# adelacvg/NS2VC

Measured on AMD Instinct MI355X. Metric: denoiser-steps/sec (10s@24kHz Vocos latent, bs32), higher is better.
Workload: dtype fp16; 1 GPU; 10 s utterance (T=938 Vocos frames), batch 32/GPU, prompt Lp=469, 20-step unipc order 2, hipGraph-captured loop, fp16 MFMA operands; timed job = set_condition + 20 steps; global_batch=32, frames=938, prompt_frames=469, solver=unipc, parallelism=dp1

## Files before the change

### include/ns2vc_hip.h

```cpp
#ifndef NS2VC_HIP_H
#define NS2VC_HIP_H

#include <stddef.h>
#include <stdint.h>

#ifdef __cplusplus
extern "C" {
#endif

#define NS2VC_ABI_VERSION 7
#define NS2VC_MAX_LEVELS 8
#define NS2VC_NCOEF 12

typedef struct ns2vc_unet ns2vc_unet;

typedef struct ns2vc_unet_cfg {
  int32_t latent_channels;
  int32_t content_channels;
  int32_t n_levels;
  int32_t block_out_channels[NS2VC_MAX_LEVELS];
  int32_t norm_num_groups;
  int32_t cross_attention_dim;
  int32_t heads;
  int32_t layers_per_block;
// ... 168 lines not shown
typedef struct ns2vc_rowchain_args {
  const void* a_op; int32_t lda;
  const void* wstream; const float* bias1; const float* consts2;
  const float* res; int32_t ldres;
  float* out1_f32; int32_t ldo1;
  void* out2_op; int32_t ldo2;
  float ln_eps; int32_t M, dim, n2;
  unsigned* ln_health;
  const float* gn_x; int32_t ldx;
  const long long* gn_stats; const float* gn_gamma; const float* gn_beta;
  float gn_eps; int32_t T, G;
  int32_t slices;
  const int32_t* lens;
} ns2vc_rowchain_args;
int ns2vc_pack_rowchain(const float* w1_host, const float* w2_host, int dim, int n2, int precision, void** out_stream_dev);
int ns2vc_pack_rowchain_sliced(const float* w1_host, const float* w2_host, int dim, int n2, int slices, int precision, void** out_stream_dev);
int ns2vc_k_rowchain(const ns2vc_rowchain_args* a, int precision, void* stream);
int ns2vc_debug_set_geglu_min_rows(int rows);
int ns2vc_debug_set_attn_keys(int keys);
int ns2vc_debug_set_attn_optimistic(int on);
int ns2vc_debug_set_attn_resident(int mode);
unsigned long long ns2vc_debug_attn_resident_launches(void);
int ns2vc_debug_attnres_table(int* rows);
int ns2vc_debug_set_rowchain_tokens(int nt);

int ns2vc_to_operand(const float* host, size_t n, int precision, void** out_dev);
int ns2vc_from_operand(const void* dev, size_t n, int precision, float* host);
int ns2vc_round_to_operand(const float* host_in, size_t n, int precision, float* host_out);
int ns2vc_pack_weight(const float* rows_host, int N, int K, int precision, void** out_dev);
int ns2vc_k_gemm(const ns2vc_gemm_args* a, int precision, void* stream);
int ns2vc_pack_conv3_tiled(const float* rows_host, int N, int ctot, int c2, int precision, void** out_dev);
int ns2vc_weight_rowsum(const float* rows_host, int N, int K, int precision, float** out_dev);
int ns2vc_debug_set_gemm_trace(void* dev_u64_blocks_x8);
int ns2vc_debug_poison(unsigned pattern, int lds_bytes, void* stream);
int ns2vc_debug_placement(void* stream, int n_blocks, int spin, uint32_t* out_host);
int ns2vc_debug_kernel_table(int family, int* rows, int* unready);
int ns2vc_debug_set_gemm_tile(int bm, int bn, int stages);
int ns2vc_k_attention(const ns2vc_attn_args* a, int head_dim, int precision, void* stream);
int ns2vc_k_groupnorm(const float* a0, int lda0, int c0, const float* a1, int lda1, int c1, int B, int T, int G, float eps,
                      const float* gamma, const float* beta, const float* temb, int ldtemb, int temb_off, int silu,
                      void* out_op, void* raw_op, int precision, void* stream);
int ns2vc_k_groupnorm_stats(const float* a0, int lda0, int c0, const long long* stats0, int B, int T, int G, float eps, const float* gamma,
                            const float* beta, const float* temb, int ldtemb, int temb_off, int silu, void* out_op, int precision, void* stream);
int ns2vc_k_groupnorm_stats2(const float* a0, int lda0, int c0, const long long* stats0, const float* a1, int lda1, int c1, const long long* stats1,
                             int B, int T, int G, float eps, const float* gamma, const float* beta, const float* temb, int ldtemb, int temb_off,
                             int silu, void* out_op, void* raw_op, int precision, void* stream);
// ... 39 lines not shown
```

### ns2vc_amd/_lib.py

```python
from __future__ import annotations

import ctypes as C
import os
from typing import Optional

_HERE = os.path.dirname(os.path.abspath(__file__))
LIB_PATH = os.path.join(_HERE, "lib", "libns2vc_hip.so")
NCOEF = 12
MAX_LEVELS = 8
PREC_F32, PREC_BF16, PREC_F16 = 0, 1, 2
ABI_VERSION = 7


class Ns2vcError(RuntimeError):
    pass


class UnetCfg(C.Structure):
    _fields_ = [
        ("latent_channels", C.c_int32), ("content_channels", C.c_int32), ("n_levels", C.c_int32),
        ("block_out_channels", C.c_int32 * MAX_LEVELS), ("norm_num_groups", C.c_int32),
        ("cross_attention_dim", C.c_int32), ("heads", C.c_int32), ("layers_per_block", C.c_int32),
        ("pool_heads", C.c_int32),
    ]
# ... 166 lines not shown
    "ns2vc_debug_set_gemm_tile": (_I, [_I, _I, _I]),
    "ns2vc_debug_kernel_table": (_I, [_I, C.POINTER(C.c_int), C.POINTER(C.c_int)]),
    "ns2vc_debug_placement": (_I, [_P, _I, _I, C.POINTER(C.c_uint32)]),
    "ns2vc_debug_poison": (_I, [C.c_uint, _I, _P]),
    "ns2vc_k_attention": (_I, [C.POINTER(AttnArgs), _I, _I, _P]),
    "ns2vc_pack_ffn": (_I, [_P, _P, _I, _I, _PP]),
    "ns2vc_pack_ffn_pre": (_I, [_P, _P, _P, _I, _I, _PP]),
    "ns2vc_xattn_pack_bytes": (C.c_size_t, [_I, _I, _I]),
    "ns2vc_k_xattn_pack": (_I, [_P, _I, _P, _I, _I, _I, _I, _P, _I, _P]),
    "ns2vc_k_ffn": (_I, [C.POINTER(FfnArgs), _I, _P]),
    "ns2vc_pack_geglu": (_I, [_P, _P, _I, _I, _PP, _PP]),
    "ns2vc_k_geglu": (_I, [C.POINTER(GegluArgs), _I, _P]),
    "ns2vc_pack_geglu_host": (_I, [_P, _P, _I, _I, _P, _P]),
    "ns2vc_debug_set_geglu_min_rows": (_I, [_I]),
    "ns2vc_pack_rowchain": (_I, [_P, _P, _I, _I, _I, _PP]),
    "ns2vc_pack_rowchain_sliced": (_I, [_P, _P, _I, _I, _I, _I, _PP]),
    "ns2vc_k_rowchain": (_I, [C.POINTER(RowchainArgs), _I, _P]),
    "ns2vc_debug_set_rowchain_tokens": (_I, [_I]),
    "ns2vc_debug_set_attn_keys": (_I, [_I]),
    "ns2vc_debug_set_attn_optimistic": (_I, [_I]),
    "ns2vc_debug_set_attn_resident": (_I, [_I]),
    "ns2vc_debug_attnres_table": (_I, [C.POINTER(_I)]),
    "ns2vc_debug_attn_resident_launches": (C.c_ulonglong, []),
    "ns2vc_k_groupnorm_stats": (_I, [_P, _I, _I, _P, _I, _I, _I, C.c_float, _P, _P, _P, _I, _I, _I, _P, _I, _P]),
    "ns2vc_k_groupnorm_stats2": (_I, [_P, _I, _I, _P, _P, _I, _I, _P, _I, _I, _I, C.c_float, _P, _P, _P, _I, _I, _I, _P, _P, _I, _P]),
    "ns2vc_k_groupnorm": (_I, [_P, _I, _I, _P, _I, _I, _I, _I, _I, C.c_float, _P, _P, _P, _I, _I, _I, _P, _P, _I, _P]),
    "ns2vc_k_layernorm_apply": (_I, [_P, _I, _I, _I, C.c_float, _P, _I, _P]),
    "ns2vc_to_operand": (_I, [_P, C.c_size_t, _I, _PP]),
    "ns2vc_from_operand": (_I, [_P, C.c_size_t, _I, _P]),
    "ns2vc_round_to_operand": (_I, [_P, C.c_size_t, _I, _P]),
    "ns2vc_k_nct_to_btc": (_I, [_P, _I, _I, _I, _P, _I, _I, _P]),
    "ns2vc_k_btc_to_nct": (_I, [_P, _I, _I, _I, _I, _P, _P]),
    "ns2vc_k_noise": (_I, [_P, _I, _I, _I, _I, _I, _P, _P, _P]),
    "ns2vc_k_solver_update": (_I, [_P, _P, _P, _P, _P, _I, _P, _P, _P, _P, C.c_size_t, _I, _P]),
    "ns2vc_k_solver_update_guided": (_I, [_P, _P, _P, _P, _P, _I, _P, _P, _P, _P, C.c_size_t, _I, _P, _I, _P, _P, _I, _P]),
    "ns2vc_k_abs_quantile": (_I, [_P, _I, _I, _I, _I, _P, C.c_float, _P, _P]),
    "ns2vc_k_solver_update_corrected": (_I, [_P, _P, _P, _P, _P, _I, _P, _P, _P, _P, C.c_size_t, _I, _I, _P, _P, _I, _I, C.c_float, C.c_float, _P, _P]),
    "ns2vc_k_solver_update_items": (_I, [_P, _I, _P, _P, _I, _P, _P, _P, _I, _P, _P, _P, _P, C.c_size_t, _I, _I, _P, _P, _P, _I, _I, C.c_float, C.c_float,
                                         _P, _P]),
    "ns2vc_k_solver_update_items_corrected": (_I, [_P, _I, _P, _P, _I, _P, _P, _P, _I, _P, _P, _P, _P, C.c_size_t, _I, _I, _P, _P, _P, _I, _P, _P, _P,
                                                   _P, _P]),
    "ns2vc_sampler_open": (_I, [_P, _I, _I, _P]),
    "ns2vc_sampler_rebase": (_I, [_P, _P]),
    "ns2vc_sampler_write_rows": (_I, [_P, _I, _I, C.POINTER(C.c_float), _P]),
    "ns2vc_sampler_admit": (_I, [_P, _I, _P, _P, _P, _P]),
    "ns2vc_sampler_take": (_I, [_P, _I, _P, _P, _P]),
# ... 48 lines not shown
```

### ns2vc_amd/csrc/abi_kernels.cpp

```cpp
#include "engine_internal.h"
#include "kernel_table.h"

#include <algorithm>
#include <cstring>
#include <mutex>

using namespace ns2vc;

hipError_t ns2vc::init_all_attributes() {
  hipError_t e = init_gemm_attributes();
  if (e == hipSuccess) e = init_convts_attributes();
  if (e == hipSuccess) e = init_attn_attributes();
  if (e == hipSuccess) e = init_attnres_attributes();
  if (e == hipSuccess) e = init_ffn_attributes();
  if (e == hipSuccess) e = init_geglu_attributes();
  if (e == hipSuccess) e = init_rowchain_attributes();
  return e;
}
static int init_attributes(hipError_t (*init)(), bool* once = nullptr) {
  if (once && *once) return 0;
  const hipError_t e = init();
  if (e != hipSuccess) return fail("kernel attribute setup failed: %s", hipGetErrorString(e));
  if (once) *once = true;
  return 0;
// ... 196 lines not shown
  static bool inited = false;
  if (init_attributes(init_rowchain_attributes, &inited)) return 1;
  std::vector<unsigned short> st;
  if (pack_rowchain_stream(w1_host, w2_host, dim, n2, precision, st, slices) != hipSuccess)
    return fail("rowchain (sliced): dim 384, n2 = dim or 3 dim, 2 slices, 16-bit precision");
  return upload_u16(st, out_stream_dev);
}
int ns2vc_debug_set_attn_keys(int keys) {
  if (keys != 0 && keys != 64 && keys != 128) return fail("attention K/V tile: 0 (heuristic), 64 or 128 keys");
  set_forced_attn_keys(keys);
  return 0;
}
int ns2vc_debug_set_attn_resident(int mode) {
  if (mode < -1 || mode > 1) return fail("resident attention: -1 (the rule), 0 (never) or 1 (whenever the launch fits)");
  set_attn_resident_mode(mode);
  return 0;
}
unsigned long long ns2vc_debug_attn_resident_launches(void) { return attn_resident_launches(); }
int ns2vc_debug_attnres_table(int* rows) {
  if (!rows) return fail("attnres table: rows not NULL");
  *rows = attnres_kernel_table().n;
  return 0;
}
int ns2vc_debug_set_rowchain_tokens(int nt) {
  if (nt < 0 || nt > 2) return fail("rowchain tokens: 0 (heuristic), 1 (64-token blocks) or 2 (128-token blocks)");
  set_forced_rowchain_tokens(nt);
  return 0;
}
int ns2vc_k_rowchain(const ns2vc_rowchain_args* a, int precision, void* stream) {
  if (!a) return fail("null args");
  return launched(launch_rowchain(*a, precision, (hipStream_t)stream), "launch_rowchain");
}
size_t ns2vc_xattn_pack_bytes(int B, int Lk, int hd) { return xattn_pack_bytes(B, Lk, hd); }
int ns2vc_k_xattn_pack(const void* k, int ldk, const void* v, int ldv, int B, int Lk, int hd, void* out, int precision, void* stream) {
  hipError_t e = launch_xattn_pack(k, ldk, v, ldv, B, Lk, hd, out, precision, (hipStream_t)stream);
  if (e != hipSuccess) return fail("xattn_pack: %s (16-bit precisions, head dim 16 | 32, 8 heads, 16-byte aligned k rows)", hipGetErrorString(e));
  return 0;
}
int ns2vc_k_ffn(const ns2vc_ffn_args* a, int precision, void* stream) {
  if (!a) return fail("null args");
  return launched(launch_ffn(*a, precision, (hipStream_t)stream), "launch_ffn");
}
int ns2vc_pack_geglu(const float* w1_packed_host, const float* bias1_packed_host, int dim, int precision, void** out_stream_dev, float** out_consts_dev) {
  if (!w1_packed_host || !out_stream_dev || !out_consts_dev) return fail("null argument");
  if (init_attributes(init_geglu_attributes)) return 1;
  std::vector<unsigned short> st;
// ... 242 lines not shown
```

### ns2vc_amd/csrc/common.h

```cpp
#pragma once
#include <hip/hip_runtime.h>
#include <stdint.h>
#include <stddef.h>
#include <vector>
#include "../../include/ns2vc_hip.h"

namespace ns2vc {

typedef __attribute__((ext_vector_type(8))) __bf16 bf16x8_t;
typedef __attribute__((ext_vector_type(16))) float f32x16_t;
typedef __attribute__((ext_vector_type(4))) float f32x4_t;
typedef __attribute__((ext_vector_type(4))) unsigned int u32x4_t;

struct bf16_t { uint16_t v; };
struct f16_t { uint16_t v; };

__host__ __device__ inline uint16_t f32_to_bf16_bits(float f) {
  union { float f; uint32_t u; } x;
  x.f = f;
  uint32_t u = x.u;
  if ((u & 0x7fffffffu) > 0x7f800000u) return (uint16_t)((u >> 16) | 0x40);
  u += 0x7fffu + ((u >> 16) & 1u);
  return (uint16_t)(u >> 16);
}
// ... 245 lines not shown
bool gemm_uses_convts(const GemmArgs& g, int prec);
int last_gemm_refusal_line();
hipError_t launch_attention(const AttnArgs& a, int head_dim, int prec, hipStream_t s, bool resident = true);
bool attention_resident_eligible(const AttnArgs& a, int head_dim, int prec, bool allow);
hipError_t launch_attention_resident(const AttnArgs& a, int head_dim, int prec, hipStream_t s);
hipError_t init_attnres_attributes();
void set_attn_resident_mode(int mode);
unsigned long long attn_resident_launches();
void set_attnres_optimistic(int on);
bool attention_masks_rows(const AttnArgs& a, int head_dim, int prec);
hipError_t init_gemm_attributes();
bool convts_eligible(const GemmArgs& g, int prec);
int convts_default_bn(const GemmArgs& g);
int convts_bn_for(const GemmArgs& g, int bn128_min);
void set_convts_bn128_min(int wgs);
int convts_row_blocks(const GemmArgs& g);
hipError_t launch_convts(const GemmArgs& g, int prec, int bn, int nl, int ks, hipStream_t s);
hipError_t init_convts_attributes();
hipError_t pack_conv3_tiled(const float* rows, int N, int ctot, int c2, int prec, std::vector<unsigned char>& out);
void set_forced_gemm_tile(int bm, int bn, int stages);
void set_gemm_trace(unsigned long long* p);
hipError_t init_attn_attributes();
void set_forced_attn_keys(int keys);
hipError_t launch_ffn(const ::ns2vc_ffn_args& a, int prec, hipStream_t s);
bool ffn_eligible(int dim, int T, int prec);
bool ffn_masks_rows(const ::ns2vc_ffn_args& a, int prec);
hipError_t init_ffn_attributes();
hipError_t pack_ffn_stream(const float* w1p, const float* w2f, const float* w0, int dim, int prec, std::vector<unsigned short>& out);
void set_ffn_trace(unsigned long long* p);
bool geglu_eligible(int dim, int T, int prec);
hipError_t pack_geglu_stream(const float* w1p, const float* bias1p, int dim, int prec, std::vector<unsigned short>& stream, std::vector<float>& consts);
hipError_t launch_geglu(const ::ns2vc_geglu_args& a, int prec, hipStream_t s);
bool geglu_masks_rows(const ::ns2vc_geglu_args& a, int prec);
hipError_t init_geglu_attributes();
void set_gg_trace(unsigned long long* p);
void set_ts_trace(unsigned long long* p);
void set_attn_optimistic(int on);

hipError_t launch_gn_partial(const float* a0, int lda0, int c0, const float* a1, int lda1, int c1,
                             int B, int T, int G, double* partial, int nchunk, int rows_per_chunk, hipStream_t s);
hipError_t launch_gn_apply(const float* a0, int lda0, int c0, const float* a1, int lda1, int c1, int B, int T, int G, float eps,
                           const double* partial, int nchunk, const long long* st0, const long long* st1, const float* gamma,
                           const float* beta, const float* temb, int ldtemb, int temb_off, int silu, void* out_op, void* raw_op,
                           int prec, hipStream_t s, int pair = 0,
                           const int* lens = nullptr);
hipError_t launch_mask_rows(void* dst, size_t ldd_bytes, size_t row_bytes, int B, int T, const int* lens, hipStream_t s, const void* src = nullptr,
                            size_t lds_bytes = 0, int Tsrc = 0, int up = 0);
hipError_t launch_ln_apply_op(const float* x, int ldx, int M, int C, float eps, void* out_op, int prec, hipStream_t s);
// ... 71 lines not shown
```

### ns2vc_amd/csrc/engine.cpp

```cpp
#include "engine_internal.h"

#include <algorithm>
#include <cstdlib>
#include <cstring>

using namespace ns2vc;

static int bind_device(ns2vc_unet* h) {
  int cur = -1;
  HIPCHK(hipGetDevice(&cur));
  if (cur != h->device) HIPCHK(hipSetDevice(h->device));
  return 0;
}
int ns2vc::check_ready(ns2vc_unet* h, bool need_plan) {
  if (!h) return fail("null engine handle");
  if (bind_device(h)) return 1;
  if (!h->finalized) return fail("weights not finalized (call ns2vc_unet_finalize_weights)");
  if (need_plan && !h->arena) return fail("engine not prepared (call ns2vc_unet_prepare)");
  return 0;
}

int ns2vc::load_state(ns2vc_unet* h, const float* x_bct, hipStream_t s, int items) {
  const int B = items > 0 ? items : h->B;
  HIPCHK(launch_nct_to_btc(x_bct, h->cfg.latent_channels, h->T, B, h->xe, h->xe_op, h->prec, h->CP, h->CP, s, h->pair_width(), h->pair_off()));
  if (!h->lens.masked) return 0;
  const size_t ob = (size_t)h->pair_width() * operand_bytes(h->prec);
  HIPCHK(launch_mask_rows(h->xe, (size_t)h->CP * 4, (size_t)h->CP * 4, B, h->T, h->lens.dev, s));
  HIPCHK(launch_mask_rows(h->xe_op, ob, ob, B, h->T, h->lens.dev, s));
  return 0;
}

static const struct { const char* name; const char* env; bool ns2vc_unet::* member; } kOptions[] = {
  {"ln_linear", "NS2VC_LN_LINEAR", &ns2vc_unet::ln_linear}, {"fold_ff", "NS2VC_FOLD_FF", &ns2vc_unet::fold_ff},
  {"fuse_ffn", "NS2VC_FUSE_FFN", &ns2vc_unet::fuse_ffn}, {"fuse_ffn_pre", "NS2VC_FUSE_FFN_PRE", &ns2vc_unet::fuse_ffn_pre},
  {"fuse_geglu", "NS2VC_FUSE_GEGLU", &ns2vc_unet::fuse_geglu}, {"fuse_rows", "NS2VC_FUSE_ROWS", &ns2vc_unet::fuse_rows},
  {"fuse_rows_gn", "NS2VC_FUSE_ROWS_GN", &ns2vc_unet::fuse_rows_gn}, {"fuse_gn_gemm", "NS2VC_FUSE_GN_GEMM", &ns2vc_unet::fuse_gn_gemm},
  {"fuse_gn_cat", "NS2VC_FUSE_GN_CAT", &ns2vc_unet::fuse_gn_cat}, {"gn_coop", "NS2VC_GN_COOP", &ns2vc_unet::gn_coop},
  {"slice_rows", "NS2VC_SLICE_ROWS", &ns2vc_unet::slice_rows}, {"attn_fp8", "NS2VC_ATTN_FP8", &ns2vc_unet::attn_fp8},
  {"attn_optimistic", "NS2VC_ATTN_OPTIMISTIC", &ns2vc_unet::attn_optimistic}, {"conv_ts", "NS2VC_CONV_TS", &ns2vc_unet::conv_ts},
  {"conv_wtiled", "NS2VC_CONV_WTILED", &ns2vc_unet::conv_wtiled}, {"gn_inloop", "NS2VC_GN_INLOOP", &ns2vc_unet::gn_inloop},
  {"fuse_solver", "NS2VC_FUSE_SOLVER", &ns2vc_unet::fuse_solver}, {"fuse_xattn", "NS2VC_FUSE_XATTN", &ns2vc_unet::fuse_xattn},
  {"fork_temb", "NS2VC_FORK_TEMB", &ns2vc_unet::fork_temb}, {"exact_io", "NS2VC_EXACT_IO", &ns2vc_unet::exact_io},
  {"split_io", "NS2VC_SPLIT_IO", &ns2vc_unet::split_io}, {"masked_fuse", "NS2VC_MASKED_FUSE", &ns2vc_unet::masked_fuse},
  {"masked_attn", "NS2VC_MASKED_ATTN", &ns2vc_unet::masked_attn}, {"masked_rows", "NS2VC_MASKED_ROWS", &ns2vc_unet::masked_rows},
  {"masked_ffn", "NS2VC_MASKED_FFN", &ns2vc_unet::masked_ffn}, {"masked_geglu", "NS2VC_MASKED_GEGLU", &ns2vc_unet::masked_geglu},
  {"attn_resident", "NS2VC_ATTN_RESIDENT", &ns2vc_unet::attn_resident}};
static bool* option_ptr(ns2vc_unet* h, const char* name) {
  for (const auto& o : kOptions)
    if (!strcmp(name, o.name)) return &(h->*o.member);
  return nullptr;
}

extern "C" {

int ns2vc_unet_create(const ns2vc_unet_cfg* cfg, ns2vc_unet** out) {
  if (!cfg || !out) return fail("null argument");
  if (cfg->n_levels < 2 || cfg->n_levels > NS2VC_MAX_LEVELS) return fail("n_levels=%d out of range (2..%d)", cfg->n_levels, NS2VC_MAX_LEVELS);
  if (cfg->latent_channels <= 0 || cfg->latent_channels > 128) return fail("latent_channels=%d must be in 1..128", cfg->latent_channels);
  if (cfg->content_channels <= 0 || cfg->content_channels % 64)
    return fail("content_channels=%d must be a positive multiple of 64", cfg->content_channels);
  if (cfg->cross_attention_dim <= 0 || cfg->cross_attention_dim % 128)
    return fail("cross_attention_dim=%d must be a positive multiple of 128", cfg->cross_attention_dim);
  if (cfg->heads < 1) return fail("heads=%d must be >= 1", cfg->heads);
  if (cfg->norm_num_groups < 1 || cfg->norm_num_groups > 8) return fail("norm_num_groups=%d unsupported (1..8)", cfg->norm_num_groups);
  if (cfg->layers_per_block < 1) return fail("layers_per_block=%d must be >= 1", cfg->layers_per_block);
  if (cfg->pool_heads < 1 || cfg->cross_attention_dim % cfg->pool_heads || cfg->cross_attention_dim / cfg->pool_heads > 8)
    return fail("cross_attention_dim=%d over pool_heads=%d: the pool head width must be a whole number <= 8", cfg->cross_attention_dim, cfg->pool_heads);
  if (cfg->block_out_channels[0] != 128) return fail("block_out_channels[0]=%d must be 128 (padded latent width)", cfg->block_out_channels[0]);
  for (int l = 0; l < cfg->n_levels; ++l) {
// ... 459 lines not shown
```

### ns2vc_amd/csrc/engine_internal.h

```cpp
#pragma once
#include "common.h"

#include <cmath>
#include <cstdarg>
#include <cstdio>
#include <cstring>
#include <functional>
#include <map>
#include <string>
#include <vector>

namespace ns2vc {

inline thread_local std::string g_err;

inline int fail(const char* fmt, ...) {
  char buf[1024];
  va_list ap;
  va_start(ap, fmt);
  vsnprintf(buf, sizeof(buf), fmt, ap);
  va_end(ap);
  g_err = buf;
  return 1;
}
// ... 212 lines not shown
  int conv_out_prec = -1;
  bool fork_temb = false;
  struct TembFork {
    int begin = -1, end = -1, join = -1;
    int first = -1, readers = 0;
    bool ok = false;
    int join_skip = 0;
    hipStream_t side_stream = nullptr;
    hipEvent_t ev_fork = nullptr, ev_join = nullptr;
  } tfork;
  bool fuse_xattn = false;
  bool fuse_solver = false;
  ns2vc::GemmArgs conv_out_g;
  int conv_out_idx = -1;
  bool warned_wtiled = false;
  int bn128_min = 160;
  bool gn_inloop = false;
  int gn_coop_min = 2;
  int cus = 256;
  int xcd_probe = -1;
  bool slice_rows = true;
  unsigned* ln_health = nullptr;
  bool attn_optimistic = true;
  bool attn_resident = true;
  unsigned* attn_fallbacks = nullptr;
  unsigned long long coef_hash = 0;
  std::vector<ns2vc::Tap> taps;
  bool has_mask = false;
  bool masked_fuse = false;
  bool masked_attn = false;
  bool masked_rows = false;
  bool masked_ffn = false;
  bool masked_geglu = false;
  struct Lengths {
    bool masked = false;
    int* dev = nullptr;
    size_t off = 0;
    float* selfbias = nullptr;
    std::vector<int32_t> applied;
    ns2vc::Staged stage;
  } lens;
  struct PromptLengths {
    bool on = false;
    int* dev = nullptr;
    std::vector<int32_t> applied;
    ns2vc::Staged stage;
// ... 111 lines not shown
```

### ns2vc_amd/csrc/ffn.hip

```cpp
#include "common.h"
#include <type_traits>
#include "mma.h"
#include "kernel_table.h"
#include <vector>

namespace ns2vc {

typedef ::ns2vc_ffn_args FfnArgs;

__device__ unsigned long long* g_ffn_trace = nullptr;
#ifndef NS2VC_GEMM_TRACE
#define NS2VC_GEMM_TRACE 0
#endif
#ifndef NS2VC_FFN_FENCE
#define NS2VC_FFN_FENCE 1
#endif
#ifndef NS2VC_FFN_WARM
#define NS2VC_FFN_WARM 1
#endif
#if NS2VC_FFN_FENCE == 1
#define FFN_FRAG_FENCE() do { asm volatile("s_waitcnt lgkmcnt(0)" ::: "memory"); __builtin_amdgcn_sched_barrier(0); } while (0)
#elif NS2VC_FFN_FENCE == 2
#define FFN_FRAG_FENCE() __builtin_amdgcn_sched_barrier(0)
#else
// ... 651 lines not shown
  return hipGetLastError();
}

static uint64_t ffn_key(const FfnArgs& a, int prec, bool masked) { return kernel_key(prec, a.dim, a.pre_a || a.att_q, a.att_q != nullptr, masked); }
#define NS2VC_FFN_ROW(TM, PREC, D, PRE, ATT, MK) \
  {kernel_key(PREC, D, PRE, ATT, MK), reinterpret_cast<const void*>(ffn_kernel<TM, D, PRE, ATT, MK>), (uint32_t)FfnGeom<D, PRE>::LDS, 512}
#define NS2VC_FFN_ROWS(PRE, ATT, MK)                                                              \
  NS2VC_FFN_ROW(bf16_t, PREC_BF16, 128, PRE, ATT, MK), NS2VC_FFN_ROW(bf16_t, PREC_BF16, 256, PRE, ATT, MK), \
  NS2VC_FFN_ROW(f16_t, PREC_F16, 128, PRE, ATT, MK), NS2VC_FFN_ROW(f16_t, PREC_F16, 256, PRE, ATT, MK)
static const KernelRow ffn_rows[] = {
  NS2VC_FFN_ROWS(false, false, false), NS2VC_FFN_ROWS(true, false, false),
  NS2VC_FFN_ROWS(false, false, true), NS2VC_FFN_ROWS(true, false, true),
  NS2VC_FFN_ROWS(true, true, false),
};
#undef NS2VC_FFN_ROWS
#undef NS2VC_FFN_ROW
static const KernelTable k_ffn_table(ffn_rows);
const KernelTable& ffn_kernel_table() { return k_ffn_table; }

bool ffn_masks_rows(const FfnArgs& a, int prec) {
  return ffn_eligible(a.dim, a.T, prec) && a.B >= 1 && a.M == a.B * a.T && find(k_ffn_table, ffn_key(a, prec, true));
}

hipError_t launch_ffn(const FfnArgs& a, int prec, hipStream_t s) {
  if (!ffn_eligible(a.dim, a.T, prec) || a.M <= 0 || a.M != a.B * a.T) return hipErrorInvalidValue;
  if (a.lens) {
    if (!ffn_masks_rows(a, prec)) return hipErrorInvalidValue;
  }
  if (!a.wstream || !a.consts || !a.bias2 || !a.res || (!a.out_f32 && !a.out_op)) return hipErrorInvalidValue;
  if (a.att_q) {
    if (!a.pre_bias || !a.pre_res || (a.pre_ldres & 3) || !a.att_kv || a.att_Lk < 1 || (a.att_ldq & 7) ||
        ((reinterpret_cast<uintptr_t>(a.att_q) | reinterpret_cast<uintptr_t>(a.att_kv)) & 15) || !(a.att_scale > 0.f))
      return hipErrorInvalidValue;
  } else if (a.pre_a ? (!a.pre_bias || !a.pre_res || (a.pre_lda & 7) || (a.pre_ldres & 3) || (unsigned long long)a.M * a.pre_lda * 2ull > 0xFFF00000ull)
              : (!a.yn || !a.ln_stats))
    return hipErrorInvalidValue;
  if ((!a.pre_a && !a.att_q && (a.ldy & 7)) || (a.ldres & 3) || (a.out_f32 && (a.ldo_f32 & 3)) || (a.out_op && (a.ldo_op & 3))) return hipErrorInvalidValue;
  if (!a.pre_a && !a.att_q && (unsigned long long)a.M * a.ldy * 2ull > 0xFFF00000ull) return hipErrorInvalidValue;
  const KernelRow* row = find(k_ffn_table, ffn_key(a, prec, a.lens != nullptr));
  if (!row) return hipErrorInvalidValue;
  return launch(*row, dim3(a.att_q ? a.B * ((a.T + 63) / 64) : (a.M + 63) / 64), s, a);
}

hipError_t init_ffn_attributes() { return set_lds_all(k_ffn_table); }

}
```

### ns2vc_amd/csrc/kernel_table.h

```cpp
#pragma once
#include <hip/hip_runtime.h>

#include <cstdint>

namespace ns2vc {

constexpr uint64_t KEY_NONE = ~0ull;
constexpr uint64_t kernel_key() { return 0; }
template <typename... I> constexpr uint64_t kernel_key(int f, I... rest) {
  static_assert(sizeof...(I) < 6, "six fields of ten bits");
  const uint64_t r = kernel_key(rest...);
  return ((unsigned)f >> 10) || r == KEY_NONE ? KEY_NONE : (r << 10 | (unsigned)f);
}

struct KernelRow {
  uint64_t key;
  const void* fn;
  uint32_t lds;
  uint32_t threads;
};
struct KernelTable {
  const KernelRow* rows;
  int n;
  template <int N> constexpr KernelTable(const KernelRow (&r)[N]) : rows(r), n(N) {}
// ... 5 lines not shown
  return nullptr;
}
inline hipError_t set_lds_all(const KernelTable& t) {
  for (int i = 0; i < t.n; ++i) {
    const hipError_t e = hipFuncSetAttribute(t.rows[i].fn, hipFuncAttributeMaxDynamicSharedMemorySize, (int)t.rows[i].lds);
    if (e != hipSuccess) return e;
  }
  return hipSuccess;
}
template <typename... A> hipError_t launch(const KernelRow& r, dim3 grid, hipStream_t s, const A&... args) {
  void* p[] = {const_cast<void*>(static_cast<const void*>(&args))...};
  (void)hipLaunchKernel(r.fn, grid, dim3(r.threads), p, r.lds, s);
  return hipGetLastError();
}

const KernelTable& gemm2_kernel_table();
const KernelTable& gemm4_kernel_table();
const KernelTable& conv3ts_kernel_table();
const KernelTable& attn_kernel_table();
const KernelTable& ffn_kernel_table();
const KernelTable& geglu_kernel_table();
const KernelTable& rowchain_kernel_table();
const KernelTable& attnres_kernel_table();

}
```

### ns2vc_amd/csrc/plan.cpp

```cpp
#include "engine_internal.h"

#include <algorithm>
#include <cmath>
#include <cstring>

namespace ns2vc {

int g_geglu_min_rows = 4608;

std::vector<int> level_lengths(int T, int n_levels) {
  std::vector<int> Ts(n_levels);
  Ts[0] = T;
  for (int l = 1; l < n_levels; ++l) Ts[l] = (Ts[l - 1] + 1) / 2;
  return Ts;
}

namespace {

struct Planner {
  ns2vc_unet* h;
  std::vector<Op>* ops;
  bool sizing = false;
  size_t off = 0;
  int B, T, Lp, G, prec;
// ... 343 lines not shown
      gemm(t + ".attn2.to_out", g);
    }
    if (ffn_ok) {
      ns2vc_ffn_args f;
      memset(&f, 0, sizeof(f));
      f.yn = yn; f.ldy = d; f.ln_stats = r3; f.ln_eps = 1e-5f;
      f.wstream = a.ffn_stream; f.consts = a.ffn_consts; f.bias2 = a.ffpo.bias;
      if (ffn_pre) {
        f.yn = nullptr; f.ln_stats = nullptr; f.wstream = a.ffn_pre_stream;
        f.pre_a = ao; f.pre_lda = d; f.pre_bias = a.o2.bias; f.pre_res = y; f.pre_ldres = d;
      }
      if (xatt) {
        f.pre_a = nullptr;
        f.att_q = qb; f.att_ldq = d; f.att_kv = xattn_vt[a.prefix];
        f.att_bias = (h->has_mask || h->plens.on) ? h->maskbias : nullptr; f.att_scale = 1.0f / std::sqrt((float)hd); f.att_Lk = Lp;
      }
      f.res = x; f.ldres = d;
      f.out_f32 = out; f.ldo_f32 = d; f.out_op = out_op; f.ldo_op = d;
      f.stats = new_stats(out, Tl, d);
      f.B = B; f.T = Tl; f.M = M; f.dim = d; f.ln_health = h->ln_health;
      if (lens_ffn) f.lens = lens_of(Tl);
      const double fl = 2.0 * M * (double)d * ((ffn_pre ? 14.0 : 13.0) * d) + (xatt ? 4.0 * B * h->cfg.heads * (double)Tl * Lp * hd : 0.0);
      add(a.prefix + (xatt ? ".ffn[attn2.sdpa+to_out+geglu+ff.out+proj_out]" : ffn_pre ? ".ffn[attn2.to_out+geglu+ff.out+proj_out]" : ".ffn[geglu+ff.out+proj_out]"),
          [=](hipStream_t s) { return launch_ffn(f, pr, s); }, 1, fl,
          (double)M * d * (opsz + 8.0 + (ffn_pre ? 4.0 : 0.0) + (out_op ? opsz : 0.0)) + (ffn_pre ? 14.0 : 13.0) * d * d * opsz +
              (xatt ? (double)opsz * B * d * 2.0 * Lp : 0.0));
      return;
    }
    auto geglu_masks = [&]() {
      ns2vc_geglu_args f;
      memset(&f, 0, sizeof(f));
      f.M = M; f.dim = d; f.T = Tl;
      return geglu_masks_rows(f, pr);
    };
    const bool lens_geglu = masked && h->masked_geglu && ops == &h->fwd_ops && level_of(Tl) >= 0 && lin_dense && fold && h->fuse_geglu &&
                            a.geglu_stream && geglu_eligible(d, Tl, pr) && M >= g_geglu_min_rows && geglu_masks();
    if (!r3 && !lens_geglu) layernorm(t + ".norm3");
    if (lens_geglu || (r3 && h->fuse_geglu && a.geglu_stream && geglu_eligible(d, Tl, pr) && M >= g_geglu_min_rows)) {
      ns2vc_geglu_args f;
      memset(&f, 0, sizeof(f));
      f.yn = yn; f.ldy = d; f.ln_stats = r3; f.ln_eps = 1e-5f;
      if (lens_geglu) { f.yn = qb; f.ln_stats = nullptr; f.T = Tl; f.lens = lens_of(Tl); }
      f.wstream = a.geglu_stream; f.consts = a.geglu_consts;
      f.out_op = ffh; f.ldo = 4 * d; f.M = M; f.dim = d; f.ln_health = h->ln_health;
      add(t + ".ff.geglu[token-stationary]", [=](hipStream_t s) { return launch_geglu(f, pr, s); }, 1, 2.0 * M * (double)d * 8.0 * d,
          (double)M * d * opsz * 5.0 + (double)M * (d / 64) * 8.0 + 8.0 * d * d * opsz);
    } else {
// ... 338 lines not shown
```

Baseline: 284.5 denoiser-steps/s (batch 32 per GPU, whole job).

## Add 128-token wide fused FFN kernel for dim-128 pre-projection path

Adds a new fused feed-forward kernel (to_out + LayerNorm + GEGLU + ff.out + proj_out) that processes 128 tokens per block with 8 waves, a 7-deep weight-tile ring in LDS and a cooperative weight prefetch. It is used when dim is 128, the pre-projection path is active without masks or cross-attention, and the 64-token grid would exceed the CU count. The aim is to halve how often the weight stream is re-read per token and raise MFMA reuse. The cost is a large LDS footprint per block, lower occupancy, and a dispatch rule that may pick the wrong kernel for some shapes.

Result: no change. 287.1 denoiser-steps/s (batch 32 per GPU, whole job), median of 6 (+0.9%).

```diff
diff --git a/include/ns2vc_hip.h b/include/ns2vc_hip.h
--- a/include/ns2vc_hip.h
+++ b/include/ns2vc_hip.h
@@ -214,6 +214,14 @@
 int ns2vc_debug_set_attn_resident(int mode);
 unsigned long long ns2vc_debug_attn_resident_launches(void);
 int ns2vc_debug_attnres_table(int* rows);
+#define NS2VC_FFNW_16BIT 1
+#define NS2VC_FFNW_PRE 2
+#define NS2VC_FFNW_LENS 4
+#define NS2VC_FFNW_ATT 8
+int ns2vc_debug_set_ffn_wide(int mode);
+unsigned long long ns2vc_debug_ffn_wide_launches(void);
+int ns2vc_debug_ffn_wide_rule(int M, int dim, int flags, int cus);
+int ns2vc_debug_ffnwide_table(int* rows);
 int ns2vc_debug_set_rowchain_tokens(int nt);
 
 int ns2vc_to_operand(const float* host, size_t n, int precision, void** out_dev);
diff --git a/ns2vc_amd/_lib.py b/ns2vc_amd/_lib.py
--- a/ns2vc_amd/_lib.py
+++ b/ns2vc_amd/_lib.py
@@ -212,6 +212,10 @@
     "ns2vc_debug_set_attn_resident": (_I, [_I]),
     "ns2vc_debug_attnres_table": (_I, [C.POINTER(_I)]),
     "ns2vc_debug_attn_resident_launches": (C.c_ulonglong, []),
+    "ns2vc_debug_set_ffn_wide": (_I, [_I]),
+    "ns2vc_debug_ffn_wide_launches": (C.c_ulonglong, []),
+    "ns2vc_debug_ffn_wide_rule": (_I, [_I, _I, _I, _I]),
+    "ns2vc_debug_ffnwide_table": (_I, [C.POINTER(_I)]),
     "ns2vc_k_groupnorm_stats": (_I, [_P, _I, _I, _P, _I, _I, _I, C.c_float, _P, _P, _P, _I, _I, _I, _P, _I, _P]),
     "ns2vc_k_groupnorm_stats2": (_I, [_P, _I, _I, _P, _P, _I, _I, _P, _I, _I, _I, C.c_float, _P, _P, _P, _I, _I, _I, _P, _P, _I, _P]),
     "ns2vc_k_groupnorm": (_I, [_P, _I, _I, _P, _I, _I, _I, _I, _I, C.c_float, _P, _P, _P, _I, _I, _I, _P, _P, _I, _P]),
diff --git a/ns2vc_amd/csrc/abi_kernels.cpp b/ns2vc_amd/csrc/abi_kernels.cpp
--- a/ns2vc_amd/csrc/abi_kernels.cpp
+++ b/ns2vc_amd/csrc/abi_kernels.cpp
@@ -242,6 +242,18 @@
   *rows = attnres_kernel_table().n;
   return 0;
 }
+int ns2vc_debug_set_ffn_wide(int mode) {
+  if (mode < -1 || mode > 1) return fail("128-token feed-forward: -1 (the rule), 0 (never) or 1 (whenever the arguments fit)");
+  set_ffn_wide_mode(mode);
+  return 0;
+}
+unsigned long long ns2vc_debug_ffn_wide_launches(void) { return ffn_wide_launches(); }
+int ns2vc_debug_ffn_wide_rule(int M, int dim, int flags, int cus) { return ffn_wide_rule(M, dim, flags, cus) ? 1 : 0; }
+int ns2vc_debug_ffnwide_table(int* rows) {
+  if (!rows) return fail("ffnwide table: rows not NULL");
+  *rows = ffnwide_kernel_table().n;
+  return 0;
+}
 int ns2vc_debug_set_rowchain_tokens(int nt) {
   if (nt < 0 || nt > 2) return fail("rowchain tokens: 0 (heuristic), 1 (64-token blocks) or 2 (128-token blocks)");
   set_forced_rowchain_tokens(nt);
diff --git a/ns2vc_amd/csrc/common.h b/ns2vc_amd/csrc/common.h
--- a/ns2vc_amd/csrc/common.h
+++ b/ns2vc_amd/csrc/common.h
@@ -291,8 +291,14 @@
 void set_gemm_trace(unsigned long long* p);
 hipError_t init_attn_attributes();
 void set_forced_attn_keys(int keys);
-hipError_t launch_ffn(const ::ns2vc_ffn_args& a, int prec, hipStream_t s);
+hipError_t launch_ffn(const ::ns2vc_ffn_args& a, int prec, hipStream_t s, bool wide = true);
 bool ffn_eligible(int dim, int T, int prec);
+bool ffn_wide_rule(int M, int dim, int flags, int cus);
+bool ffn_wide_eligible(const ::ns2vc_ffn_args& a, int prec, bool allow);
+hipError_t launch_ffn_wide(const ::ns2vc_ffn_args& a, int prec, hipStream_t s);
+hipError_t init_ffnwide_attributes();
+void set_ffn_wide_mode(int mode);
+unsigned long long ffn_wide_launches();
 bool ffn_masks_rows(const ::ns2vc_ffn_args& a, int prec);
 hipError_t init_ffn_attributes();
 hipError_t pack_ffn_stream(const float* w1p, const float* w2f, const float* w0, int dim, int prec, std::vector<unsigned short>& out);
diff --git a/ns2vc_amd/csrc/engine.cpp b/ns2vc_amd/csrc/engine.cpp
--- a/ns2vc_amd/csrc/engine.cpp
+++ b/ns2vc_amd/csrc/engine.cpp
@@ -44,7 +44,7 @@
   {"split_io", "NS2VC_SPLIT_IO", &ns2vc_unet::split_io}, {"masked_fuse", "NS2VC_MASKED_FUSE", &ns2vc_unet::masked_fuse},
   {"masked_attn", "NS2VC_MASKED_ATTN", &ns2vc_unet::masked_attn}, {"masked_rows", "NS2VC_MASKED_ROWS", &ns2vc_unet::masked_rows},
   {"masked_ffn", "NS2VC_MASKED_FFN", &ns2vc_unet::masked_ffn}, {"masked_geglu", "NS2VC_MASKED_GEGLU", &ns2vc_unet::masked_geglu},
-  {"attn_resident", "NS2VC_ATTN_RESIDENT", &ns2vc_unet::attn_resident}};
+  {"attn_resident", "NS2VC_ATTN_RESIDENT", &ns2vc_unet::attn_resident}, {"ffn_wide", "NS2VC_FFN_WIDE", &ns2vc_unet::ffn_wide}};
 static bool* option_ptr(ns2vc_unet* h, const char* name) {
   for (const auto& o : kOptions)
     if (!strcmp(name, o.name)) return &(h->*o.member);
diff --git a/ns2vc_amd/csrc/engine_internal.h b/ns2vc_amd/csrc/engine_internal.h
--- a/ns2vc_amd/csrc/engine_internal.h
+++ b/ns2vc_amd/csrc/engine_internal.h
@@ -258,6 +258,7 @@
   bool slice_rows = true;
   unsigned* ln_health = nullptr;
   bool attn_optimistic = true;
+  bool ffn_wide = true;
   bool attn_resident = true;
   unsigned* attn_fallbacks = nullptr;
   unsigned long long coef_hash = 0;
diff --git a/ns2vc_amd/csrc/ffn.hip b/ns2vc_amd/csrc/ffn.hip
--- a/ns2vc_amd/csrc/ffn.hip
+++ b/ns2vc_amd/csrc/ffn.hip
@@ -697,7 +697,7 @@
   return ffn_eligible(a.dim, a.T, prec) && a.B >= 1 && a.M == a.B * a.T && find(k_ffn_table, ffn_key(a, prec, true));
 }
 
-hipError_t launch_ffn(const FfnArgs& a, int prec, hipStream_t s) {
+hipError_t launch_ffn(const FfnArgs& a, int prec, hipStream_t s, bool wide) {
   if (!ffn_eligible(a.dim, a.T, prec) || a.M <= 0 || a.M != a.B * a.T) return hipErrorInvalidValue;
   if (a.lens) {
     if (!ffn_masks_rows(a, prec)) return hipErrorInvalidValue;
@@ -714,9 +714,13 @@
   if (!a.pre_a && !a.att_q && (unsigned long long)a.M * a.ldy * 2ull > 0xFFF00000ull) return hipErrorInvalidValue;
   const KernelRow* row = find(k_ffn_table, ffn_key(a, prec, a.lens != nullptr));
   if (!row) return hipErrorInvalidValue;
+  if (ffn_wide_eligible(a, prec, wide)) return launch_ffn_wide(a, prec, s);
   return launch(*row, dim3(a.att_q ? a.B * ((a.T + 63) / 64) : (a.M + 63) / 64), s, a);
 }
 
-hipError_t init_ffn_attributes() { return set_lds_all(k_ffn_table); }
-
-}
+hipError_t init_ffn_attributes() {
+  const hipError_t e = set_lds_all(k_ffn_table);
+  return e != hipSuccess ? e : init_ffnwide_attributes();
+}
+
+}
diff --git a/ns2vc_amd/csrc/ffn_wide.hip b/ns2vc_amd/csrc/ffn_wide.hip
--- /dev/null
+++ b/ns2vc_amd/csrc/ffn_wide.hip
@@ -0,0 +1,419 @@
+#include "common.h"
+#include "mma.h"
+#include "kernel_table.h"
+
+#include <atomic>
+
+namespace ns2vc {
+
+typedef ::ns2vc_ffn_args FfnArgs;
+
+#ifndef NS2VC_FFN_WARM
+#define NS2VC_FFN_WARM 1
+#endif
+#ifndef NS2VC_FFNW_ABLATE
+#define NS2VC_FFNW_ABLATE 0
+#endif
+#define FFNW_FRAG_FENCE() do { asm volatile("s_waitcnt lgkmcnt(0)" ::: "memory"); __builtin_amdgcn_sched_barrier(0); } while (0)
+
+constexpr int FFNW_TILE = 128 * 128;
+
+struct FfnWideGeom {
+  static constexpr int D = 128, TOK = 128;
+  static constexpr int RING = 7;
+  static constexpr int KT = D / 64, NB = D / 32, NSS = D / 32;
+  static constexpr int TILES = KT + NSS * (2 * KT + 2) + KT;
+  static constexpr int PANEL = KT * TOK * 128;
+  static constexpr int CONSTS = 8 * D * 8;
+  static constexpr int XCH = TOK * 4 * 8;
+  static constexpr int LDS = RING * FFNW_TILE + PANEL + CONSTS + XCH;
+  static_assert(LDS <= 160 * 1024, "LDS budget");
+  static constexpr int EP = 36;
+  static_assert(4 * 4 * 32 * EP * 4 <= RING * FFNW_TILE, "epilogue staging (one 32-channel block) fits in the ring");
+  static_assert(2 * NB * 512 * 8 <= PANEL, "per-lane statistics partials of both halves fit in the panel");
+};
+
+template <typename TM>
+__global__ __launch_bounds__(512) void ffnwide_kernel(const FfnArgs a) {
+  op_mode_init<TM>();
+  using G = FfnWideGeom;
+  constexpr int D = G::D, KT = G::KT, NB = G::NB, NSS = G::NSS, NT = G::TILES, EP = G::EP, RING = G::RING, PT = G::TOK * 128;
+  extern __shared__ __attribute__((aligned(16))) char smem[];
+  char* const ring = smem;
+  char* const panel = smem + RING * FFNW_TILE;
+  const float* const consts = reinterpret_cast<const float*>(panel + G::PANEL);
+
+  const int tid = threadIdx.x, lane = tid & 63;
+  const int wave = __builtin_amdgcn_readfirstlane(tid >> 6);
+  const int tq = wave & 3, hp = wave >> 2;
+  const int l31 = lane & 31, hi = lane >> 5;
+  const int sw = (l31 >> 1) & 7;
+  const unsigned lds0 = (unsigned)(size_t)smem;
+  const int m0 = (int)blockIdx.x * G::TOK, mlim = a.M;
+  const int tok = 32 * tq + l31, mtok = m0 + tok;
+
+  const i32x4_t rW = make_rsrc(a.wstream, (NS2VC_FFNW_ABLATE & 1) ? 0ull : (unsigned long long)NT * FFNW_TILE);
+  const unsigned lane16 = (unsigned)(lane * 16);
+#if NS2VC_FFN_WARM
+  {
+    const unsigned nx = (gridDim.x + 7) >> 3, jx = blockIdx.x >> 3;
+    const unsigned total = (unsigned)NT * FFNW_TILE;
+    const unsigned per = (((total + nx - 1) / nx) + 8191u) & ~8191u;
+    for (unsigned off = jx * per + wave * 1024; off < min(total, (jx + 1) * per); off += 8192)
+      blds16(rW, lane16, off, lds0 + (RING - 1) * FFNW_TILE + wave * 1024);
+  }
+#endif
+  {
+    const i32x4_t rY = make_rsrc(a.pre_a, (unsigned long long)a.M * a.pre_lda * 2ull);
+#pragma unroll
+    for (int h = 0; h < 2; ++h) {
+      const int prow = 64 * h + 8 * wave + (lane >> 3), pchunk = lane & 7;
+      const int m = m0 + prow;
+      const unsigned voff = m < mlim ? (unsigned)m * (unsigned)a.pre_lda * 2u + (unsigned)((pchunk ^ ((prow >> 1) & 7)) * 16) : DMA_OOB;
+#pragma unroll
+      for (int kt = 0; kt < KT; ++kt) blds16(rY, voff, (unsigned)(kt * 128), lds0 + RING * FFNW_TILE + kt * PT + (8 * h + wave) * 1024);
+    }
+    const i32x4_t rC = make_rsrc(a.consts, (unsigned long long)G::CONSTS);
+    blds16(rC, lane16, (unsigned)(wave * 1024), lds0 + RING * FFNW_TILE + G::PANEL + wave * 1024);
+  }
+  float4 b0[2][4], rr0[2][4];
+#pragma unroll
+  for (int g2 = 0; g2 < 2; ++g2)
+#pragma unroll
+    for (int g = 0; g < 4; ++g) {
+      const int n = 32 * (hp + 2 * g2) + 8 * g + 4 * hi;
+      b0[g2][g] = *reinterpret_cast<const float4*>(a.pre_bias + n);
+      rr0[g2][g] = mtok < mlim ? *reinterpret_cast<const float4*>(a.pre_res + (size_t)mtok * a.pre_ldres + n) : make_float4(0.f, 0.f, 0.f, 0.f);
+    }
+  auto issue_tile = [&](int p) __attribute__((always_inline)) {
+    const int slot = p % RING, r = (p + 6 - KT) % 6;
+    const int src = (p >= KT && p < NT - KT && (r == 1 || r == 2)) ? p + 3 - 2 * r : p;
+#pragma unroll
+    for (int j = 0; j < 2; ++j)
+      blds16(rW, lane16, (unsigned)(src * FFNW_TILE + (j * 8 + wave) * 1024), lds0 + slot * FFNW_TILE + (j * 8 + wave) * 1024);
+  };
+#pragma unroll
+  for (int q = 0; q < RING - 2; ++q) issue_tile(q);
+
+  float mean = 0.f, rstd = 1.f;
+  auto ln_finish = [&](float s, float q) __attribute__((always_inline)) {
+    const float inv = 1.0f / (float)D;
+    mean = s * inv;
+    double var = (double)q * (double)inv - (double)mean * (double)mean;
+    if (var < 0.0) var = 0.0;
+    rstd = 1.0f / sqrtf((float)var + a.ln_eps);
+    if (a.ln_health && hp == 0) {
+      float ratio = mtok < mlim ? fabsf(mean) * rstd : 0.f;
+#pragma unroll
+      for (int o = 32; o > 0; o >>= 1) ratio = fmaxf(ratio, __shfl_xor(ratio, o));
+      if (lane == 0 && ratio > __uint_as_float(__hip_atomic_load(a.ln_health, __ATOMIC_RELAXED, __HIP_MEMORY_SCOPE_AGENT)))
+        atomicMax(a.ln_health, __float_as_uint(ratio));
+    }
+  };
+
+  int p = 0;
+  auto step_begin = [&](bool first = false) __attribute__((always_inline)) {
+    const int after = min(RING - 4, NT - 2 - p);
+    if (after >= 3) wait_vmcnt<6>();
+    else if (after == 2) wait_vmcnt<4>();
+    else if (after == 1) wait_vmcnt<2>();
+    else wait_vmcnt<0>();
+    asm volatile("s_waitcnt lgkmcnt(0)" ::: "memory");
+    __builtin_amdgcn_s_barrier();
+    if (first) {
+#pragma unroll
+      for (int g2 = 0; g2 < 2; ++g2)
+#pragma unroll
+        for (int g = 0; g < 4; ++g) {
+          asm volatile("" : "+v"(b0[g2][g].x), "+v"(b0[g2][g].y), "+v"(b0[g2][g].z), "+v"(b0[g2][g].w));
+          asm volatile("" : "+v"(rr0[g2][g].x), "+v"(rr0[g2][g].y), "+v"(rr0[g2][g].z), "+v"(rr0[g2][g].w));
+        }
+    }
+    if (p + RING - 2 < NT) issue_tile(p + RING - 2);
+    if (p + RING - 1 < NT) issue_tile(p + RING - 1);
+  };
+  auto tile = [&](int q) __attribute__((always_inline)) -> const char* { return ring + (q % RING) * FFNW_TILE; };
+  const char* const bpanel = panel + tok * 128;
+
+  {
+    f32x16_t acc0[2];
+#pragma unroll
+    for (int i = 0; i < 2; ++i)
+#pragma unroll
+      for (int r = 0; r < 16; ++r) acc0[i][r] = 0.f;
+    step_begin(true);
+    {
+#pragma unroll
+      for (int kt = 0; kt < KT; ++kt) {
+        const char* T = tile(p + kt);
+        u32x4_t fb[4], fw[2][4];
+#pragma unroll
+        for (int ks = 0; ks < 4; ++ks) {
+          const int c = ((2 * ks + hi) ^ sw) * 16;
+          fb[ks] = *reinterpret_cast<const u32x4_t*>(bpanel + kt * PT + c);
+#pragma unroll
+          for (int g2 = 0; g2 < 2; ++g2) fw[g2][ks] = *reinterpret_cast<const u32x4_t*>(T + (32 * (hp + 2 * g2) + l31) * 128 + c);
+        }
+#pragma unroll
+        for (int ks = 0; ks < 4; ++ks)
+#pragma unroll
+          for (int g2 = 0; g2 < 2; ++g2) MmaT<TM>::mma(acc0[g2], fw[g2][ks], fb[ks]);
+      }
+      p += KT;
+    }
+    asm volatile("s_waitcnt lgkmcnt(0)" ::: "memory");
+    __builtin_amdgcn_s_barrier();
+    float2* const xch = reinterpret_cast<float2*>(panel + G::PANEL + G::CONSTS);
+#pragma unroll
+    for (int g2 = 0; g2 < 2; ++g2) {
+      const int hw = hp + 2 * g2;
+      float ps = 0.f, pq = 0.f;
+#pragma unroll
+      for (int g = 0; g < 4; ++g) {
+        float4 v;
+        v.x = acc0[g2][4 * g + 0] + b0[g2][g].x + rr0[g2][g].x;
+        v.y = acc0[g2][4 * g + 1] + b0[g2][g].y + rr0[g2][g].y;
+        v.z = acc0[g2][4 * g + 2] + b0[g2][g].z + rr0[g2][g].z;
+        v.w = acc0[g2][4 * g + 3] + b0[g2][g].w + rr0[g2][g].w;
+        if (mtok >= mlim) v = make_float4(0.f, 0.f, 0.f, 0.f);
+        ps += (v.x + v.y) + (v.z + v.w);
+        pq += (v.x * v.x + v.y * v.y) + (v.z * v.z + v.w * v.w);
+        const int n = 32 * hw + 8 * g + 4 * hi;
+        char* dst = panel + (n >> 6) * PT + tok * 128 + ((((n & 63) >> 3) ^ sw) * 16) + 8 * hi;
+        *reinterpret_cast<uint2*>(dst) = make_uint2(Op16<TM>::pack(v.x, v.y), Op16<TM>::pack(v.z, v.w));
+      }
+      const auto s2 = __builtin_amdgcn_permlane32_swap(__float_as_uint(ps), __float_as_uint(ps), false, false);
+      const auto q2 = __builtin_amdgcn_permlane32_swap(__float_as_uint(pq), __float_as_uint(pq), false, false);
+      ps = __uint_as_float(s2[0]) + __uint_as_float(s2[1]);
+      pq = __uint_as_float(q2[0]) + __uint_as_float(q2[1]);
+      if (hi == 0) xch[tok * 4 + hw] = make_float2(ps, pq);
+    }
+    __syncthreads();
+    float s = 0.f, q = 0.f;
+#pragma unroll
+    for (int k = 0; k < 4; ++k) { const float2 v = xch[tok * 4 + k]; s += v.x; q += v.y; }
+    ln_finish(s, q);
+  }
+
+  f32x16_t accO[2][NB];
+#pragma unroll
+  for (int g2 = 0; g2 < 2; ++g2)
+#pragma unroll
+    for (int i = 0; i < NB; ++i)
+#pragma unroll
+      for (int r = 0; r < 16; ++r) accO[g2][i][r] = 0.f;
+
+#pragma unroll
+  for (int ss = 0; ss < NSS; ++ss) {
+    u32x4_t hf[2][2];
+#pragma unroll
+    for (int g2 = 0; g2 < 2; ++g2) {
+      f32x16_t av, ag;
+#pragma unroll
+      for (int r = 0; r < 16; ++r) { av[r] = 0.f; ag[r] = 0.f; }
+      step_begin();
+      {
+        u32x4_t fb[3], fv[3], fg[3];
+        auto load = [&](int b) __attribute__((always_inline)) {
+          const char* wrow = tile(p + (b >> 2)) + (64 * hp + l31) * 128;
+          const int c = ((2 * (b & 3) + hi) ^ sw) * 16;
+          fb[b % 3] = *reinterpret_cast<const u32x4_t*>(bpanel + (b >> 2) * PT + c);
+          fv[b % 3] = *reinterpret_cast<const u32x4_t*>(wrow + c);
+          fg[b % 3] = *reinterpret_cast<const u32x4_t*>(wrow + 32 * 128 + c);
+        };
+        load(0);
+        load(1);
+#pragma unroll
+        for (int b = 0; b < 4 * KT; ++b) {
+          __builtin_amdgcn_sched_barrier(0);
+          if (b + 2 < 4 * KT) load(b + 2);
+          __builtin_amdgcn_sched_barrier(0);
+          MmaT<TM>::mma(av, fv[b % 3], fb[b % 3]);
+          MmaT<TM>::mma(ag, fg[b % 3], fb[b % 3]);
+        }
+        __builtin_amdgcn_sched_barrier(0);
+        p += KT;
+      }
+      const float* cv = consts + (size_t)(256 * ss + 64 * (hp + 2 * g2)) * 2;
+#pragma unroll
+      for (int s = 0; s < 2; ++s) {
+        float h[8];
+#pragma unroll
+        for (int j = 2 * s; j < 2 * s + 2; ++j) {
+          const float4 v0 = *reinterpret_cast<const float4*>(cv + (8 * j + 4 * hi) * 2);
+          const float4 v1 = *reinterpret_cast<const float4*>(cv + (8 * j + 4 * hi) * 2 + 4);
+          const float4 g0 = *reinterpret_cast<const float4*>(cv + (32 + 8 * j + 4 * hi) * 2);
+          const float4 g1 = *reinterpret_cast<const float4*>(cv + (32 + 8 * j + 4 * hi) * 2 + 4);
+          const float wsv[4] = {v0.x, v0.z, v1.x, v1.z}, bv[4] = {v0.y, v0.w, v1.y, v1.w};
+          const float wsg[4] = {g0.x, g0.z, g1.x, g1.z}, bg[4] = {g0.y, g0.w, g1.y, g1.w};
+#pragma unroll
+          for (int i = 0; i < 4; ++i) {
+            const float pv = rstd * (av[4 * j + i] - mean * wsv[i]) + bv[i];
+            const float pg = rstd * (ag[4 * j + i] - mean * wsg[i]) + bg[i];
+            h[4 * (j - 2 * s) + i] = (NS2VC_FFNW_ABLATE & 2) ? pv * pg : pv * gelu_erf_f(pg);
+          }
+        }
+        hf[g2][s] = u32x4_t{Op16<TM>::pack(h[0], h[1]), Op16<TM>::pack(h[2], h[3]), Op16<TM>::pack(h[4], h[5]), Op16<TM>::pack(h[6], h[7])};
+        __builtin_amdgcn_sched_barrier(0);
+      }
+    }
+    step_begin();
+    {
+      u32x4_t fw[2][2][4];
+      auto load = [&](int g2) __attribute__((always_inline)) {
+        const char* wrow = tile(p + g2) + l31 * 128;
+#pragma unroll
+        for (int s = 0; s < 2; ++s)
+#pragma unroll
+          for (int i = 0; i < 4; ++i)
+            fw[g2][s][i] = *reinterpret_cast<const u32x4_t*>(wrow + i * 32 * 128 + ((4 * hp + 2 * s + hi) ^ sw) * 16);
+      };
+      load(0);
+#pragma unroll
+      for (int g2 = 0; g2 < 2; ++g2) {
+        FFNW_FRAG_FENCE();
+        if (g2 == 0) load(1);
+        __builtin_amdgcn_sched_barrier(0);
+#pragma unroll
+        for (int s = 0; s < 2; ++s)
+#pragma unroll
+          for (int i = 0; i < 4; ++i) MmaT<TM>::mma(accO[g2][i], fw[g2][s][i], hf[g2][s]);
+      }
+      p += 2;
+    }
+  }
+  step_begin();
+#pragma unroll
+  for (int kt = 0; kt < KT; ++kt) {
+    const char* T = tile(p + kt);
+#pragma unroll
+    for (int g2 = 0; g2 < 2; ++g2) {
+      const int c = ((2 * (hp + 2 * g2) + hi) ^ sw) * 16;
+      const u32x4_t b = *reinterpret_cast<const u32x4_t*>(bpanel + kt * PT + c);
+#pragma unroll
+      for (int i = 0; i < 4; ++i) {
+        const u32x4_t w = *reinterpret_cast<const u32x4_t*>(T + (32 * i + l31) * 128 + c);
+        MmaT<TM>::mma(accO[g2][i], w, b);
+      }
+    }
+  }
+  p += KT;
+
+  __syncthreads();
+  float* const E = reinterpret_cast<float*>(ring);
+  float2* const P = reinterpret_cast<float2*>(panel);
+  const int L = tid, eth = L >> 8, etok = (L >> 3) & 31, equad = L & 7;
+  float4 rr[2][NB];
+#pragma unroll
+  for (int hh = 0; hh < 2; ++hh) {
+    const int em = m0 + 64 * hh + 32 * eth + etok;
+#pragma unroll
+    for (int nb = 0; nb < NB; ++nb) {
+      rr[hh][nb] = em < mlim ? *reinterpret_cast<const float4*>(a.res + (size_t)em * a.ldres + 32 * nb + 4 * equad) : make_float4(0.f, 0.f, 0.f, 0.f);
+      const float4 bb = *reinterpret_cast<const float4*>(a.bias2 + 32 * nb + 4 * equad);
+      rr[hh][nb].x += bb.x; rr[hh][nb].y += bb.y; rr[hh][nb].z += bb.z; rr[hh][nb].w += bb.w;
+    }
+  }
+  TM* const oo = reinterpret_cast<TM*>(a.out_op);
+#pragma unroll
+  for (int nb = 0; nb < NB; ++nb) {
+    if (nb) lds_barrier();
+#pragma unroll
+    for (int g2 = 0; g2 < 2; ++g2) {
+      float* const Ew = E + ((tq * 4 + hp + 2 * g2) * 32 + l31) * EP + 4 * hi;
+#pragma unroll
+      for (int j = 0; j < 4; ++j)
+        *reinterpret_cast<float4*>(Ew + 8 * j) = make_float4(accO[g2][nb][4 * j], accO[g2][nb][4 * j + 1], accO[g2][nb][4 * j + 2], accO[g2][nb][4 * j + 3]);
+    }
+    lds_barrier();
+#pragma unroll
+    for (int hh = 0; hh < 2; ++hh) {
+      const int em = m0 + 64 * hh + 32 * eth + etok;
+      const float* const Er = E + ((2 * hh + eth) * 4 * 32 + etok) * EP + 4 * equad;
+      float4 v = *reinterpret_cast<const float4*>(Er);
+#pragma unroll
+      for (int k = 1; k < 4; ++k) {
+        const float4 w = *reinterpret_cast<const float4*>(Er + k * 32 * EP);
+        v.x += w.x; v.y += w.y; v.z += w.z; v.w += w.w;
+      }
+      const int n = 32 * nb + 4 * equad;
+      float ps = 0.f, pq = 0.f;
+      if (em < mlim) {
+        v.x += rr[hh][nb].x; v.y += rr[hh][nb].y; v.z += rr[hh][nb].z; v.w += rr[hh][nb].w;
+        if (a.out_f32) out_f4(a.out_f32 + (size_t)em * a.ldo_f32 + n, v.x, v.y, v.z, v.w);
+        if (oo) out_op4<TM>(oo + (size_t)em * a.ldo_op + n, v.x, v.y, v.z, v.w);
+        ps = (v.x + v.y) + (v.z + v.w); pq = (v.x * v.x + v.y * v.y) + (v.z * v.z + v.w * v.w);
+      }
+      if (a.stats) P[(hh * NB + nb) * 512 + L] = make_float2(ps, pq);
+    }
+  }
+  if (a.stats) {
+    lds_barrier();
+    const int blk = wave, tl = lane;
+#pragma unroll
+    for (int hh = 0; hh < 2; ++hh) {
+      const int mh = m0 + 64 * hh;
+      if (mh >= a.M) break;
+      const int bi = mh / a.T;
+      const int mB = (bi + 1) * a.T;
+      float s0 = 0.f, q0 = 0.f, s1 = 0.f, q1 = 0.f;
+      {
+        const int t64 = tl;
+        const float2* pp = P + (hh * NB + (blk >> 1)) * 512 + (t64 >> 5) * 256 + (t64 & 31) * 8 + 4 * (blk & 1);
+        float ss = 0.f, qq = 0.f;
+#pragma unroll
+        for (int c = 0; c < 4; ++c) { const float2 v = pp[c]; ss += v.x; qq += v.y; }
+        if (mh + t64 < mB) { s0 += ss; q0 += qq; } else { s1 += ss; q1 += qq; }
+      }
+#pragma unroll
+      for (int o = 1; o < 64; o <<= 1) { s0 += __shfl_xor(s0, o); q0 += __shfl_xor(q0, o); s1 += __shfl_xor(s1, o); q1 += __shfl_xor(q1, o); }
+      if (tl == 0) {
+        unsigned long long* st = reinterpret_cast<unsigned long long*>(a.stats) + ((size_t)bi * (D / 16) + blk) * 2;
+        atomicAdd(st, (unsigned long long)llrint((double)s0 * GN_SUM_SCALE));
+        atomicAdd(st + 1, (unsigned long long)llrint((double)q0 * GN_SQ_SCALE));
+        if (mB < a.M && mB < mh + 64) {
+          atomicAdd(st + 2 * (D / 16), (unsigned long long)llrint((double)s1 * GN_SUM_SCALE));
+          atomicAdd(st + 2 * (D / 16) + 1, (unsigned long long)llrint((double)q1 * GN_SQ_SCALE));
+        }
+      }
+    }
+  }
+}
+
+#define NS2VC_FFNWIDE_ROW(TM, PREC) {kernel_key(PREC, FfnWideGeom::D), reinterpret_cast<const void*>(ffnwide_kernel<TM>), (uint32_t)FfnWideGeom::LDS, 512}
+static const KernelRow ffnwide_rows[] = {NS2VC_FFNWIDE_ROW(bf16_t, PREC_BF16), NS2VC_FFNWIDE_ROW(f16_t, PREC_F16)};
+#undef NS2VC_FFNWIDE_ROW
+static const KernelTable k_ffnwide_table(ffnwide_rows);
+const KernelTable& ffnwide_kernel_table() { return k_ffnwide_table; }
+static int g_cus = 256;
+hipError_t init_ffnwide_attributes() {
+  int dev = 0, cus = 0;
+  if (hipGetDevice(&dev) == hipSuccess && hipDeviceGetAttribute(&cus, hipDeviceAttributeMultiprocessorCount, dev) == hipSuccess && cus > 0) g_cus = cus;
+  return set_lds_all(k_ffnwide_table);
+}
+
+static int g_wide_mode = -1;
+void set_ffn_wide_mode(int mode) { g_wide_mode = mode; }
+
+bool ffn_wide_rule(int M, int dim, int flags, int cus) {
+  if (flags != (NS2VC_FFNW_16BIT | NS2VC_FFNW_PRE) || dim != FfnWideGeom::D || M <= 0 || cus < 0) return false;
+  return (M + 63) / 64 > cus;
+}
+bool ffn_wide_eligible(const FfnArgs& a, int prec, bool allow) {
+  if (!allow || g_wide_mode == 0) return false;
+  const int flags = ((prec == PREC_BF16 || prec == PREC_F16) ? NS2VC_FFNW_16BIT : 0) | (a.pre_a ? NS2VC_FFNW_PRE : 0) | (a.lens ? NS2VC_FFNW_LENS : 0) |
+                    ((a.att_q || a.att_kv || a.att_bias) ? NS2VC_FFNW_ATT : 0);
+  return ffn_wide_rule(a.M, a.dim, flags, g_wide_mode == 1 ? 0 : g_cus) && find(k_ffnwide_table, kernel_key(prec, a.dim));
+}
+
+static std::atomic<unsigned long long> g_wide_launches{0};
+unsigned long long ffn_wide_launches() { return g_wide_launches.load(); }
+
+hipError_t launch_ffn_wide(const FfnArgs& a, int prec, hipStream_t s) {
+  const KernelRow* row = find(k_ffnwide_table, kernel_key(prec, a.dim));
+  if (!row) return hipErrorInvalidValue;
+  ++g_wide_launches;
+  return launch(*row, dim3((a.M + FfnWideGeom::TOK - 1) / FfnWideGeom::TOK), s, a);
+}
+
+}
diff --git a/ns2vc_amd/csrc/kernel_table.h b/ns2vc_amd/csrc/kernel_table.h
--- a/ns2vc_amd/csrc/kernel_table.h
+++ b/ns2vc_amd/csrc/kernel_table.h
@@ -51,5 +51,6 @@
 const KernelTable& geglu_kernel_table();
 const KernelTable& rowchain_kernel_table();
 const KernelTable& attnres_kernel_table();
+const KernelTable& ffnwide_kernel_table();
 
 }
diff --git a/ns2vc_amd/csrc/plan.cpp b/ns2vc_amd/csrc/plan.cpp
--- a/ns2vc_amd/csrc/plan.cpp
+++ b/ns2vc_amd/csrc/plan.cpp
@@ -389,7 +389,7 @@
       if (lens_ffn) f.lens = lens_of(Tl);
       const double fl = 2.0 * M * (double)d * ((ffn_pre ? 14.0 : 13.0) * d) + (xatt ? 4.0 * B * h->cfg.heads * (double)Tl * Lp * hd : 0.0);
       add(a.prefix + (xatt ? ".ffn[attn2.sdpa+to_out+geglu+ff.out+proj_out]" : ffn_pre ? ".ffn[attn2.to_out+geglu+ff.out+proj_out]" : ".ffn[geglu+ff.out+proj_out]"),
-          [=](hipStream_t s) { return launch_ffn(f, pr, s); }, 1, fl,
+          [=, wide = h->ffn_wide](hipStream_t s) { return launch_ffn(f, pr, s, wide); }, 1, fl,
           (double)M * d * (opsz + 8.0 + (ffn_pre ? 4.0 : 0.0) + (out_op ? opsz : 0.0)) + (ffn_pre ? 14.0 : 13.0) * d * d * opsz +
               (xatt ? (double)opsz * B * d * 2.0 * Lp : 0.0));
       return;
```
